# JuanTarrio/rebvo

Measured on AMD Instinct MI355X. Metric: frames/sec (DoG+extract+track+depth) 752x480 EuRoC, higher is better.
Workload: dtype f32 scale-space / f64 tracker+EKF

## Files before the change

### rebvo_amd/csrc/api.hip

```cpp

#include <math.h>
#include <stdio.h>
#include <stdlib.h>
#include <string.h>

#include <algorithm>
#include <mutex>

#include "ctx.h"
#include "stage_a_dev.h"

namespace edgehip {

static thread_local std::string g_err;

int wait_pinned_ring(edgehip_ctx *c) {
    const int r = c->frames_seen % 8;
    if (c->ring_valid[r]) EH_CHECK(hipEventSynchronize(c->ev_ring[r]));
    return 0;
}

static int wait_idx_row(edgehip_ctx *c, int slot, const int32_t *pi) {
    if (c->slot_src[slot].idx_row != pi) return 0;
    if (c->a_api_valid[slot]) EH_CHECK(hipEventSynchronize(c->ev_a[slot]));
// ... 379 lines not shown
        c->use_valid[i] = false;
    }
    EH_CHECK(hipEventCreateWithFlags(&c->ev_tmp, hipEventDisableTiming));
    EH_CHECK(hipEventCreateWithFlags(&c->ev_stage, hipEventDisableTiming));
    EH_CHECK(hipEventCreateWithFlags(&c->ev_stage8, hipEventDisableTiming));
    for (int i = 0; i < 8; i++) { EH_CHECK(hipEventCreateWithFlags(&c->ev_ring[i], hipEventDisableTiming)); c->ring_valid[i] = false; }
    if (nslots > 4) { set_error("edgehip_create: at most 4 frame slots"); return EDGEHIP_ERR_ARG; }

    DevicePlan &pl = c->plan;
    pl.w = p.w; pl.h = p.h; pl.n = p.w * p.h; pl.nseq = nseq; pl.nslots = nslots;
    pl.ftx = (p.w + 3) / 4;
    pl.fstride = (size_t)pl.ftx * (size_t)((p.h + 3) / 4) * 16;
    pl.f16tx = (p.w + 7) / 8;
    pl.f16stride = (size_t)pl.f16tx * (size_t)((p.h + 3) / 4) * 32;
    pl.cap = std::min(p.max_points, EDGEHIP_KEYLINE_MAX);
    const double sr0 = kovesi_boxes(p.sigma0, kMaxBoxes, pl.box[0]);
    kovesi_boxes(sr0 * p.ksigma, kMaxBoxes, pl.box[1]);
    for (int f = 0; f < 2; f++)
        for (int i = 0; i < kMaxBoxes; i++) {
            if (pl.box[f][i] < 1 || pl.box[f][i] * pl.box[f][i] >= kDivLutMax) {
                set_error("edgehip_create: box width out of range for these sigmas");
                return EDGEHIP_ERR_ARG;
            }
            pl.box_a[f][i] = (float)(1.0 / (pl.box[f][i] * pl.box[f][i]));
        }
    pl.ppx = (float)p.ppx; pl.ppy = (float)p.ppy; pl.zfx = (float)p.zfx; pl.zfy = (float)p.zfy;
    pl.zfm = (double)((pl.zfx + pl.zfy) / 2);

    const size_t B = nseq, S = nslots, N = pl.n, CAP = pl.cap;
    int e;
#define EH_TRY(x) if ((e = (x)) != 0) return e
    EH_TRY(dmalloc(c, &c->rgb, S * B * N * 3 + 16, al->dev, 0));
    EH_TRY(dmalloc(c, &c->ii, 4 * B * N, al->dev, 0));
    c->planes = nullptr;
    if (p.debug_planes) EH_TRY(dmalloc(c, &c->planes, 5 * B * N, al->dev, 0));
    EH_TRY(dmalloc(c, &c->mask, S * B * N, al->dev, 0xFF));
    EH_TRY(dmalloc(c, &c->field, B * pl.fstride, al->dev, 0xFF));
    EH_TRY(dmalloc(c, &c->field16, B * pl.f16stride, al->dev, 0));
    c->field32_valid = false;
    c->und_base = nullptr;
    c->und_iw = nullptr;
    if (p.use_undistort) {
        EH_TRY(dmalloc(c, &c->und_base, N, al->dev));
        EH_TRY(dmalloc(c, &c->und_iw, N, al->dev));
        std::vector<int32_t> base;
        std::vector<uint32_t> iw;
        build_undistort_map(p, base, iw, nullptr, nullptr);
        EH_CHECK(hipMemcpy(c->und_base, base.data(), sizeof(int32_t) * N, hipMemcpyHostToDevice));
        EH_CHECK(hipMemcpy(c->und_iw, iw.data(), sizeof(uint32_t) * 4 * N, hipMemcpyHostToDevice));
    }
    EH_TRY(dmalloc(c, &c->div_lut, kDivLutMax, al->dev));
    EH_TRY(dmalloc(c, &c->pinv, 3 * 49, al->dev, 0));
    EH_TRY(dmalloc(c, &c->seq, B, al->dev, 0));
    EH_TRY(dmalloc(c, &c->seqa, B, al->dev, 0));
    EH_TRY(dmalloc(c, &c->tresh_slot, S * B, al->dev, 0));
    c->fc_rows = std::max<int>(nslots, kRefRing);
    c->fc_index = 0;
    EH_TRY(dmalloc(c, &c->framecount, (size_t)c->fc_rows * B, al->dev, 0));
    EH_TRY(dmalloc(c, &c->kn_slot, S * B, al->dev, 0));
    EH_TRY(dmalloc(c, &c->retuned_slot, S * B, al->dev, 0));
    c->band_rows = detect_band_rows(p.w, p.plane_fit_size);
    c->nbands = (p.h - 2 * p.plane_fit_size + c->band_rows - 1) / c->band_rows;
    {
        const int npx = c->band_rows * p.w, nchunk = (npx + 63) / 64, cpw = (nchunk + kDetWaves - 1) / kDetWaves;
        c->band_cap = cpw * 64;
    }
    const size_t nstrips = (size_t)c->nbands * kDetWaves;
    EH_TRY(dmalloc(c, &c->band_cnt, B * nstrips, al->dev, 0));
    EH_TRY(dmalloc(c, &c->band_off, B * (nstrips + 1), al->dev, 0));
    {
        char *bs;
        EH_TRY(dmalloc(c, &bs, B * nstrips * c->band_cap * 20, al->dev));
        c->band_stage = bs;
    }
    EH_TRY(dmalloc(c, &c->histo, B * 256, al->dev, 0));
    c->nblk_tvr = (int)((CAP + kTvrBlock - 1) / kTvrBlock);
    EH_TRY(dmalloc(c, &c->P0, B * 3 * CAP, al->dev, 0));
    EH_TRY(dmalloc(c, &c->resid, (size_t)kResidBufs * B * CAP, al->dev, 0));
    EH_TRY(dmalloc(c, &c->resid_carry, (size_t)kResidBufs * B * c->nblk_tvr, al->dev, 0));
    EH_TRY(dmalloc(c, &c->partials, 2 * B * c->nblk_tvr * kNumSums, al->dev, 0));
    EH_TRY(dmalloc(c, &c->block_last, 2 * B * c->nblk_tvr, al->dev, 0));
    EH_TRY(dmalloc(c, &c->bin_cnt, B * 256, al->dev, 0));
    {
        const size_t ntiles = (size_t)((p.w + 63) / 64) * ((p.h + 63) / 64);
        EH_TRY(dmalloc(c, &c->bins, B * ntiles * CAP, al->dev));
    }
    c->field_radius = p.search_range;
    c->field_mode = EH_EXP_ENV("EDGEHIP_FIELD_MODE", 0);
    c->no_grec = getenv("EDGEHIP_NO_GREC") && atoi(getenv("EDGEHIP_NO_GREC")) != 0;
    c->level_mode = getenv("EDGEHIP_LEVEL_MODE") ? atoi(getenv("EDGEHIP_LEVEL_MODE")) : 0;
    c->fwd_mode = EH_EXP_ENV("EDGEHIP_FWD_MODE", 0);
    c->fused_min_batch = fused_min_env;
    c->fused_undist = EH_EXP_ENV("EDGEHIP_FUSED_UNDIST", 0) != 0;
    c->tvr_rw2 = EH_EXP_ENV("EDGEHIP_TVR_RW2", 0);
    c->dual_init = getenv("EDGEHIP_DUAL_INIT") ? atoi(getenv("EDGEHIP_DUAL_INIT")) : 1;
    c->persist_lm_max = EH_EXP_ENV("EDGEHIP_PERSIST_LM", 0);
    EH_TRY(dmalloc(c, &c->sync_cnt, B, al->dev, 0));
    EH_TRY(dmalloc(c, &c->fwd_key, B * CAP, al->dev, 0));
    EH_TRY(dmalloc(c, &c->fwd_win, B * CAP, al->dev, 0xFF));
    EH_TRY(dmalloc(c, &c->rs_tmp, B * 2 * CAP, al->dev, 0));
    c->fuse_match = !(getenv("EDGEHIP_FUSE_MATCH") && atoi(getenv("EDGEHIP_FUSE_MATCH")) == 0);
    if (c->fuse_match) {
        EH_TRY(dmalloc(c, &c->rot_pm, S * B * CAP, al->dev, 0)); EH_TRY(dmalloc(c, &c->rot_mm, S * B * CAP, al->dev, 0));
        EH_TRY(dmalloc(c, &c->rot_rho, S * B * CAP, al->dev, 0)); EH_TRY(dmalloc(c, &c->rot_srho, S * B * CAP, al->dev, 0));
    }
    EH_TRY(dmalloc(c, &c->rot_buf, B * 9, al->dev, 0));
    EH_TRY(dmalloc(c, &c->nav_dev, B, al->dev, 0));
    EH_TRY(dmalloc(c, &c->idx_dev, B, al->dev, 0));
    c->slot_src.assign(S, edgehip_ctx::SlotSrc());
    c->stereo_cnt = nullptr;
    if (p.stereo_available) EH_TRY(dmalloc(c, &c->stereo_cnt, B, al->dev, 0));
    c->nav_log = nullptr;
    c->nav_log_len = 0;

    {
        const size_t al256 = 256;
        auto up = [&](size_t x) { return (x + al256 - 1) / al256 * al256; };
        const bool stereo = p.stereo_available != 0;
        const size_t per = up(CAP * 4) * 8  +
                           up(CAP * 8) * 6  + up(CAP * 8) * 7  + up(CAP * 32) + up(CAP * 16)  +
                           (stereo ? up(CAP * 4) + 2 * up(CAP * 8) : 0);
        char *arena;
        EH_TRY(dmalloc(c, &arena, per * S * B, al->dev, 0));
        c->kl_arena = arena;
        c->kl.resize(S * B);
        for (size_t sb = 0; sb < S * B; sb++) {
            char *q = arena + sb * per;
            KlSoA &k = c->kl[sb];
            auto take = [&](size_t bytes) { char *r = q; q += up(bytes); return r; };
            k.p_inx = (int32_t *)take(CAP * 4);
            k.m_m = (float2 *)take(CAP * 8); k.u_m = (float2 *)take(CAP * 8); k.c_p = (float2 *)take(CAP * 8);
            k.p_m = (float2 *)take(CAP * 8); k.p_m_0 = (float2 *)take(CAP * 8); k.m_m0 = (float2 *)take(CAP * 8);
            k.n_m = (float *)take(CAP * 4);
            k.rho = (double *)take(CAP * 8); k.s_rho = (double *)take(CAP * 8); k.rho_nr = (double *)take(CAP * 8);
            k.s_rho_nr = (double *)take(CAP * 8); k.rho0 = (double *)take(CAP * 8); k.s_rho0 = (double *)take(CAP * 8);
            k.n_m0 = (double *)take(CAP * 8);
            k.m_id = (int32_t *)take(CAP * 4); k.m_id_f = (int32_t *)take(CAP * 4); k.m_id_kf = (int32_t *)take(CAP * 4);
            k.m_num = (int32_t *)take(CAP * 4); k.p_id = (int32_t *)take(CAP * 4); k.n_id = (int32_t *)take(CAP * 4);
            k.rec = (MatchRec *)take(CAP * 32);
            k.grec = (float4 *)take(CAP * 16);
            k.stereo_m_id = nullptr; k.stereo_rho = nullptr; k.stereo_s_rho = nullptr;
            if (stereo) {
                k.stereo_m_id = (int32_t *)take(CAP * 4);
                k.stereo_rho = (double *)take(CAP * 8); k.stereo_s_rho = (double *)take(CAP * 8);
            }
        }
        c->slot_cam.assign(S, edgehip_ctx::SlotCam{pl.ppx, pl.ppy, pl.zfm});
        EH_TRY(dmalloc(c, &c->kl_dev, S * B, al->dev));
        EH_CHECK(hipMemcpyAsync(c->kl_dev, c->kl.data(), sizeof(KlSoA) * S * B, hipMemcpyHostToDevice, c->stream));
    }
    {
        std::vector<float> lut(kDivLutMax, 0.f);
        for (int k = 1; k < kDivLutMax; k++) lut[k] = (float)(1.0 / (double)(float)k);
        EH_CHECK(hipMemcpyAsync(c->div_lut, lut.data(), sizeof(float) * kDivLutMax, hipMemcpyHostToDevice, c->stream));
        double pinv[3 * 49] = {0};
        plane_fit_pinv(p.plane_fit_size, pinv);
        if (p.plane_fit_size == 2)
            for (int i = 0; i < 5; i++)
                for (int j = 0; j < 5; j++) {
                    const int k = i * 5 + j;
                    if (!(pinv[k] == pinv[j] && pinv[25 + k] == pinv[25 + 5 * i] && pinv[50 + k] == pinv[50])) {
                        set_error("edgehip_create: plane-fit pseudo inverse lost its separable structure");
                        return EDGEHIP_ERR_STATE;
                    }
                }
        memcpy(c->pinv_host, pinv, sizeof c->pinv_host);
        EH_CHECK(hipMemcpyAsync(c->pinv, pinv, sizeof pinv, hipMemcpyHostToDevice, c->stream));
// ... 979 lines not shown
```

### rebvo_amd/csrc/ctx.h

```cpp
#pragma once
#include <hip/hip_runtime.h>
#include <stdint.h>
#include <string.h>
#include <string>
#include <map>
#include <vector>
#include <mutex>
#include <atomic>

#include "edgehip.h"
#include "export_ring.h"

namespace edgehip {

constexpr int kMaxBoxes = 3;
constexpr int kBandRows = 12;
constexpr int kDetWaves = 16;
constexpr int kDivLutMax = 256;
constexpr int kTvrThreads = 256;
constexpr int kTvrBlock = kTvrThreads;
constexpr int kNumSums = 28;
constexpr int kRefRing = 8;
constexpr int kResidBufs = 3;

__host__ __device__ inline uint64_t resid_carry_bits() { return 0x7FF8C0DEC0DEC0DEull; }

struct __attribute__((aligned(16))) MatchRec {
    float c_px, c_py, u_mx, u_my, m_mx, m_my, n_m, pad;
};

struct KlSoA {
    int32_t *p_inx;
    float2 *m_m, *u_m, *c_p, *p_m, *p_m_0, *m_m0;
    float *n_m;
    double *rho, *s_rho, *rho_nr, *s_rho_nr, *rho0, *s_rho0, *n_m0;
    int32_t *m_id, *m_id_f, *m_id_kf, *m_num, *p_id, *n_id;
    MatchRec *rec;
    float4 *grec;
    int32_t *stereo_m_id;
    double *stereo_rho, *stereo_s_rho;
};

struct SeqDev {
    edgehip_seq_state pub;
    int32_t kn_new;
    int32_t band_trunc;
    float nm_max, nm_min;
    double tresh_used;
    double X[6], Xnew[6], Xt[6], h[6];
    double JtJ[36], JtF[6], JtJnew[36], JtFnew[6];
    double F, Fnew, F0, Ft, F0t, u, v, ut, vt, gain;
    int32_t eff_steps, eff_steps_t, res_cur, res_new, res_t, lm_phase;
    int32_t kn_old, pad1;
    double s_rho_min_eval;
    double Rt[9], Vt[3], RM[4];
    int32_t nmatch_tmp, kf_tmp;
    double zX[6], zXnew[6], zh[6];
    double zJtJ[36], zJtF[6], zJtJnew[36], zJtFnew[6];
    double zF, zFnew, zF0, zu, zv, zgain;
    double zRt[9], zVt[3], zRM[4];
    int32_t z_eff_steps, z_pad;
    double mv_V[3], mv_Vnew[3], mv_h[3], mv_JtJ[9], mv_JtF[3], mv_JtJnew[9], mv_JtFnew[3], mv_RVel[9];
    double mv_F, mv_Fnew, mv_u, mv_v, mv_s_rho_min;
    float mv_min_mod; int32_t mv_pad;
    int32_t skip_match, skip_map;
    double t_cur;
    double V_track[3], W_track[3], PV_track[9], PW_track[9];
};

struct SeqA {
    double tresh;
    double tresh_used;
    int32_t l_kl_num;
    int32_t kn_new;
    int32_t band_trunc, pad0;
    float nm_max, nm_min;
    float retuned, pad1;
};

struct DevicePlan {
    int w, h, n, cap, nseq, nslots;
    int ftx;
    size_t fstride;
    int f16tx;
    size_t f16stride;
    int box[2][kMaxBoxes];
    float box_a[2][kMaxBoxes];
    float ppx, ppy, zfx, zfy;
    double zfm;
};

__device__ __forceinline__ int x86_cvttsd2si(double f) {
    if (!(f > -2147483649.0 && f < 2147483648.0)) return (int)0x80000000;
    return (int)f;
}

__device__ __forceinline__ int cvt_trunc_sat_i32(double f) {
    int r;
    asm("v_cvt_i32_f64 %0, %1" : "=v"(r) : "v"(f));
    return r;
}

#ifndef EDGEHIP_FASTDIV
#define EDGEHIP_FASTDIV 1
#endif
__device__ __forceinline__ double rcp_nr(const double b) {
// ... 528 lines not shown
```

### rebvo_amd/csrc/stage_b.hip

```cpp

#include <math.h>
#include <string.h>

#include <vector>

#include <type_traits>

#include "ctx.h"
#include "resid_carry.h"
#include "wave_reduce.h"

namespace edgehip {

struct RetuneArgs {
    SeqA *seqa;
    const int32_t *histo;
    float *retuned_out;
    int knum, nbins;
};
template <int NT>
__global__ __launch_bounds__(NT) void k_quantile(const KlSoA *kls, const int32_t *__restrict__ kns, SeqDev *seqs,
                                                 double smin, double smax, double pct, int nbins, const double *__restrict__ t_in, double fps,
                                                 RetuneArgs rt) {
    __shared__ int s_h[256];
// ... 99 lines not shown
constexpr int FT = 64;
constexpr int FG = 12;

__global__ __launch_bounds__(256) void k_field_tiles(const KlSoA *kls, const int32_t *__restrict__ masks,
                                                     const float *__restrict__ retuned, uint32_t *__restrict__ field,
                                                     int w, int h, size_t fstride, int ftx, int radius, float min_mod_arg) {
    __shared__ uint32_t s_tile[FT * FT];
    __shared__ int s_list[4096];
    __shared__ int s_cnt;
    const int seq = blockIdx.z, tid = threadIdx.x, lane = tid & 63;
    const int tx0 = blockIdx.x * FT, ty0 = blockIdx.y * FT;
    const KlSoA &k = kls[seq];
    const int32_t *mask = masks + (size_t)seq * ((size_t)w * h);
    const float min_mod = min_mod_arg < 0.f ? retuned[seq] : min_mod_arg;
    for (int i = tid; i < FT * FT; i += 256) s_tile[i] = 0xFFFFFFFFu;
    if (tid == 0) s_cnt = 0;
    const int rx0 = max(tx0 - radius - 1, 0), rx1 = min(tx0 + FT + radius + 1, w);
    const int ry0 = max(ty0 - radius - 1, 0), ry1 = min(ty0 + FT + radius + 1, h);
    const int rw = rx1 - rx0;
    const int rows_per_fill = max(1, min(FG, 4096 / rw));
    __syncthreads();
    for (int yg = ry0; yg < ry1; yg += rows_per_fill) {
        const int ye = min(yg + rows_per_fill, ry1);
        const int npx = (ye - yg) * rw;
        for (int base = 0; base < npx; base += 256) {
            const int idx = base + tid;
            int id = -1;
            if (idx < npx) {
                const int yy = yg + idx / rw, xx = rx0 + idx % rw;
                id = mask[(size_t)yy * w + xx];
            }
            const unsigned long long bal = __ballot(id >= 0);
            int wbase = 0;
            if (lane == 0 && bal) wbase = atomicAdd(&s_cnt, __popcll(bal));
            wbase = __shfl(wbase, 0, 64);
            if (id >= 0) s_list[wbase + __popcll(bal & ((1ull << lane) - 1ull))] = id;
        }
        __syncthreads();
        const int cnt = s_cnt;
        for (int li = tid; li < cnt; li += 256) {
            const int ikl = s_list[li];
            const MatchRec r = k.rec[ikl];
            if (min_mod > 0 && r.n_m < min_mod) continue;
            float tlo = (float)(-radius), thi = (float)(radius - 1);
            const float bx0 = (float)tx0 - 1.f - r.c_px, bx1 = (float)(tx0 + FT) - r.c_px;
            const float by0 = (float)ty0 - 1.f - r.c_py, by1 = (float)(ty0 + FT) - r.c_py;
            if (fabsf(r.u_mx) > 1e-6f) {
                const float a = bx0 / r.u_mx, b = bx1 / r.u_mx;
                tlo = fmaxf(tlo, fminf(a, b) - 1.f);
                thi = fminf(thi, fmaxf(a, b) + 1.f);
            } else if (bx0 > 0.f || bx1 < 0.f) continue;
            if (fabsf(r.u_my) > 1e-6f) {
                const float a = by0 / r.u_my, b = by1 / r.u_my;
                tlo = fmaxf(tlo, fminf(a, b) - 1.f);
                thi = fminf(thi, fmaxf(a, b) + 1.f);
            } else if (by0 > 0.f || by1 < 0.f) continue;
            const int t0 = (int)floorf(tlo), t1 = (int)ceilf(thi);
            const uint32_t idk = (uint32_t)(0xFFFF - ikl);
            for (int t = max(t0, -radius); t <= min(t1, radius - 1); t++) {
                const float fx = r.u_mx * (float)t + r.c_px;
                const float fy = r.u_my * (float)t + r.c_py;
                const int xi = round_half_away_i(fx), yi = round_half_away_i(fy);
                if (xi >= w || yi >= h || xi < 0 || yi < 0) continue;
                const int lx = xi - tx0, ly = yi - ty0;
                if ((unsigned)lx >= (unsigned)FT || (unsigned)ly >= (unsigned)FT) continue;
                const uint32_t at = (uint32_t)(t < 0 ? -t : t);
                atomicMin(&s_tile[ly * FT + lx], (at << 16) | idk);
            }
        }
        __syncthreads();
        if (tid == 0) s_cnt = 0;
        __syncthreads();
    }
    uint32_t *out = field + (size_t)seq * fstride;
    for (int i = tid; i < FT * FT; i += 256) {
        const int st = i >> 4, in = i & 15;
        const int lx = ((st % (FT / 4)) << 2) | (in & 3), ly = ((st / (FT / 4)) << 2) | (in >> 2);
        const int x = tx0 + lx, y = ty0 + ly;
        if (x < w && y < h) out[field_index(x, y, ftx)] = s_tile[ly * FT + lx];
    }
}

constexpr int kMaxTiles = 256;

__device__ __forceinline__ bool tile_trange(const MatchRec &r, int tx0, int ty0, int radius, int &t0, int &t1) {
    float tlo = (float)(-radius), thi = (float)(radius - 1);
    const float bx0 = (float)tx0 - 0.51f - r.c_px, bx1 = (float)(tx0 + FT) - 0.49f - r.c_px;
    const float by0 = (float)ty0 - 0.51f - r.c_py, by1 = (float)(ty0 + FT) - 0.49f - r.c_py;
    if (fabsf(r.u_mx) > 1e-6f) {
        const float iu = __builtin_amdgcn_rcpf(r.u_mx);
        const float a = bx0 * iu, b = bx1 * iu, sl = 0.25f + 1e-4f * fabsf(iu);
        tlo = fmaxf(tlo, fminf(a, b) - sl);
        thi = fminf(thi, fmaxf(a, b) + sl);
    } else if (bx0 > 0.f || bx1 < 0.f) return false;
    if (fabsf(r.u_my) > 1e-6f) {
        const float iu = __builtin_amdgcn_rcpf(r.u_my);
        const float a = by0 * iu, b = by1 * iu, sl = 0.25f + 1e-4f * fabsf(iu);
        tlo = fmaxf(tlo, fminf(a, b) - sl);
        thi = fminf(thi, fmaxf(a, b) + sl);
    } else if (by0 > 0.f || by1 < 0.f) return false;
    t0 = max((int)ceilf(tlo), -radius);
    t1 = min((int)floorf(thi), radius - 1);
    return t0 <= t1;
}

constexpr int kPackedRadiusMax = 127;
constexpr int kRngSlots = 9;

__device__ __forceinline__ uint32_t pack_trange(int t0, int t1, int radius) {
    return (uint32_t)(t0 + radius) | ((uint32_t)(t1 + radius) << 8);
}

template <bool PACKED>
__global__ __launch_bounds__(256) void k_field_bin(const KlSoA *kls, const int32_t *__restrict__ kns,
                                                   const float *__restrict__ retuned, int32_t *__restrict__ bin_cnt,
                                                   int32_t *__restrict__ bins, int w, int h, int radius, float min_mod_arg,
                                                   int ntx, int nty, int bin_cap, unsigned long long *__restrict__ fwd_key,
                                                   int32_t *__restrict__ fwd_win) {
    __shared__ int s_cnt[kMaxTiles], s_base[kMaxTiles];
    __shared__ uint16_t s_rng[PACKED ? kRngSlots * 256 : 1];
    const int seq = blockIdx.z, tid = threadIdx.x;
    const int i = blockIdx.x * 256 + tid;
    const int kn = kns[seq];
    if (blockIdx.x * 256 >= kn) return;

    const int ntiles = ntx * nty;
    for (int t = tid; t < ntiles; t += 256) s_cnt[t] = 0;
    __syncthreads();
    bool active = i < kn;
    MatchRec r;
    int txa = 0, txb = -1, tya = 0, tyb = -1;
    if (active) {
        r = kls[seq].rec[i];
        const float min_mod = min_mod_arg < 0.f ? retuned[seq] : min_mod_arg;
        if (min_mod > 0 && r.n_m < min_mod) active = false;
    }
    if (active) {
        const float rr = (float)radius + 1.5f;
        const float xa = r.c_px - fabsf(r.u_mx) * rr - 1.f, xb = r.c_px + fabsf(r.u_mx) * rr + 1.f;
        const float ya = r.c_py - fabsf(r.u_my) * rr - 1.f, yb = r.c_py + fabsf(r.u_my) * rr + 1.f;
        txa = max((int)floorf(xa) / FT, 0); txb = min((int)floorf(xb) / FT, ntx - 1);
        tya = max((int)floorf(ya) / FT, 0); tyb = min((int)floorf(yb) / FT, nty - 1);
        if (xb < 0.f || yb < 0.f) txb = -1;
    }
    const int bw = txb - txa + 1;
    const bool cached = bw > 0 && (tyb - tya + 1) * bw <= (PACKED ? kRngSlots : 32);
    uint32_t hitmask = 0;
    for (int ty = tya; ty <= tyb; ty++)
        for (int tx = txa; tx <= txb; tx++) {
            int t0, t1;
            const bool hit = tile_trange(r, tx * FT, ty * FT, radius, t0, t1);
            if (hit) atomicAdd(&s_cnt[ty * ntx + tx], 1);
            if constexpr (PACKED) {
                if (cached) s_rng[((ty - tya) * bw + (tx - txa)) * 256 + tid] = hit ? (uint16_t)pack_trange(t0, t1, radius) : (uint16_t)0xFFFFu;
            } else {
                if (hit && cached) hitmask |= 1u << ((ty - tya) * bw + (tx - txa));
            }
        }
    __syncthreads();
    for (int t = tid; t < ntiles; t += 256) {
        const int c = s_cnt[t];
        s_base[t] = c ? atomicAdd(&bin_cnt[(size_t)seq * kMaxTiles + t], c) : 0;
        s_cnt[t] = 0;
    }
    __syncthreads();
    for (int ty = tya; ty <= tyb; ty++)
        for (int tx = txa; tx <= txb; tx++) {
            int t0, t1;
            bool hit;
            uint32_t entry = (uint32_t)i;
            if constexpr (PACKED) {
                uint32_t rng;
                if (cached) { rng = s_rng[((ty - tya) * bw + (tx - txa)) * 256 + tid]; hit = rng != 0xFFFFu; }
                else { hit = tile_trange(r, tx * FT, ty * FT, radius, t0, t1); rng = hit ? pack_trange(t0, t1, radius) : 0u; }
                entry |= rng << 16;
            } else {
                hit = cached ? ((hitmask >> ((ty - tya) * bw + (tx - txa))) & 1u) != 0u : tile_trange(r, tx * FT, ty * FT, radius, t0, t1);
            }
            if (hit) {
                const int t = ty * ntx + tx;
                const int pos = s_base[t] + atomicAdd(&s_cnt[t], 1);
                if (pos < bin_cap) bins[((size_t)seq * ntiles + t) * bin_cap + pos] = (int32_t)entry;
            }
        }
    if (fwd_key && i < kn) { fwd_key[(size_t)seq * bin_cap + i] = 0ull; fwd_win[(size_t)seq * bin_cap + i] = -1; }
}

#ifndef EDGEHIP_NT_RASTER
#define EDGEHIP_NT_RASTER 1
#endif
template <bool PACKED>
__global__ __launch_bounds__(256) void k_field_raster(const KlSoA *kls, int32_t *__restrict__ bin_cnt,
                                                      const int32_t *__restrict__ bins, uint32_t *__restrict__ field,
                                                      uint16_t *__restrict__ field16, size_t f16stride, int f16tx, int keep32,
                                                      int w, int h, size_t fstride, int ftx, int radius, int ntx, int bin_cap) {
#ifndef EDGEHIP_RASTER_PAD
#define EDGEHIP_RASTER_PAD 2
#endif
    constexpr int TS = FT + EDGEHIP_RASTER_PAD;
    __shared__ uint32_t s_tile[FT * TS];
    const int ntiles = ntx * gridDim.y;
    const int seq = blockIdx.z, tid = threadIdx.x;
    const int tx0 = blockIdx.x * FT, ty0 = blockIdx.y * FT;
    const int tile = blockIdx.y * ntx + blockIdx.x;
    for (int i = tid; i < FT * TS; i += 256) s_tile[i] = 0xFFFFFFFFu;
    __syncthreads();
    const int cnt = min(bin_cnt[(size_t)seq * kMaxTiles + tile], bin_cap);
    const int32_t *list = bins + ((size_t)seq * ntiles + tile) * bin_cap;
    const KlSoA &k = kls[seq];
    const unsigned ex = (unsigned)min(FT, w - tx0), ey = (unsigned)min(FT, h - ty0);
#ifndef EDGEHIP_FSPLIT
#define EDGEHIP_FSPLIT 2
#endif
#ifndef EDGEHIP_RASTER_ABL
#define EDGEHIP_RASTER_ABL 0
#endif
#ifndef EDGEHIP_RASTER_UNROLL
#define EDGEHIP_RASTER_UNROLL 2
#endif
    constexpr int FSPLIT = EDGEHIP_FSPLIT;
    const unsigned ex4 = ex << 2;
    const int neg4tx0 = -4 * tx0;
    const unsigned org = (unsigned)(neg4tx0 - ty0 * (TS * 4));
    const float radius_f = (float)radius;
    auto raster = [&](auto fix_x, auto fix_y) {
        for (int wi = tid; wi < cnt * FSPLIT; wi += 256) {
            const int li = wi / FSPLIT, part = wi - li * FSPLIT;
            const uint32_t entry = (uint32_t)list[li];
            const int ikl = PACKED ? (int)(entry & 0xFFFFu) : (int)entry;
#if EDGEHIP_RASTER_ABL >= 5
            MatchRec r;
            r.c_px = (float)(tx0 + (ikl & 63)); r.c_py = (float)(ty0 + ((ikl >> 6) & 63)); r.u_mx = 0.6f; r.u_my = 0.8f;
#else
            MatchRec r;
            { const float4 q = ldg(reinterpret_cast<const float4 *>(k.rec), 2 * (size_t)ikl); r.c_px = q.x; r.c_py = q.y; r.u_mx = q.z; r.u_my = q.w; }
#endif
            float lo, hi;
            if constexpr (PACKED) {
                lo = (float)((entry >> 16) & 0xFFu) - radius_f;
                hi = (float)(entry >> 24) - radius_f;
            } else {
                int t0, t1;
                if (!tile_trange(r, tx0, ty0, radius, t0, t1)) continue;
                lo = (float)t0; hi = (float)t1;
            }
#ifndef EDGEHIP_RASTER_PK
#define EDGEHIP_RASTER_PK 0
#endif
#if EDGEHIP_RASTER_PK
            typedef float v2f __attribute__((ext_vector_type(2)));
            const v2f u2 = {r.u_mx, r.u_my}, c2 = {r.c_px, r.c_py};
#endif
            auto at = [&](const float tf, float &fx, float &fy) __attribute__((always_inline)) {
#if EDGEHIP_RASTER_PK
                const v2f t2 = {tf, tf};
                const v2f f2 = u2 * t2 + c2;
                fx = f2.x; fy = f2.y;
#else
                fx = r.u_mx * tf + r.c_px;
                fy = r.u_my * tf + r.c_py;
#endif
            };
            auto inside = [&](const float tf) __attribute__((always_inline)) -> bool {
                float fx, fy;
                at(tf, fx, fy);
                const int rx = decltype(fix_x)::value ? round_half_away_i(fx) : round_ties_up_i(fx);
                const int ry = decltype(fix_y)::value ? round_half_away_i(fy) : round_ties_up_i(fy);
                return (unsigned)((rx << 2) + neg4tx0) < ex4 && (unsigned)(ry - ty0) < ey;
            };
            if constexpr (FSPLIT == 2) {
                const float step = part ? -1.f : 1.f;
                float tf = part ? hi : lo;
                for (float n = hi - lo; n >= 0.f && !inside(tf); n -= 1.f) tf += step;
                const float other = __int_as_float(__builtin_amdgcn_update_dpp(0, __float_as_int(tf), 0xB1, 0xf, 0xf, true));
                lo = part ? other : tf;
                hi = part ? tf : other;
            } else {
                while (lo <= hi && !inside(lo)) lo += 1.f;
                while (hi > lo && !inside(hi)) hi -= 1.f;
            }
            if (lo > hi) continue;
            int t0 = (int)lo, t1 = (int)hi;
            {
                const int chunk = (t1 - t0 + FSPLIT) / FSPLIT;
                t0 += part * chunk;
                t1 = min(t1, t0 + chunk - 1);
            }
            const uint32_t idk = (uint32_t)(0xFFFF - ikl);
#if EDGEHIP_RASTER_ABL == 2
            uint32_t acc_abl = 0;
#endif
#if EDGEHIP_RASTER_ABL >= 3
            if (t0 == 12345) s_tile[0] = idk;
            continue;
#endif
            auto sample = [&](const float tf) __attribute__((always_inline)) {
                float fx, fy;
                at(tf, fx, fy);
                const unsigned off = ((unsigned)round_ties_up_i(fx) << 2) + (__umul24((unsigned)round_ties_up_i(fy), (unsigned)(TS * 4)) + org);
                const uint32_t val = __builtin_amdgcn_cvt_pk_u8_f32(fabsf(tf), 2u, idk);
                uint32_t *const px = reinterpret_cast<uint32_t *>(reinterpret_cast<char *>(s_tile) + off);
#if EDGEHIP_RASTER_ABL == 1
                *px = val;
#elif EDGEHIP_RASTER_ABL == 2
                acc_abl += val | off;
#else
                atomicMin(px, val);
#endif
            };
            constexpr int UNROLL = EDGEHIP_RASTER_UNROLL;
            const float t1f = (float)t1;
            float tf = (float)t0;
            if constexpr (UNROLL > 1) {
                for (; tf + (float)(UNROLL - 1) <= t1f; tf += (float)UNROLL) {
#pragma unroll
                    for (int j = 0; j < UNROLL; j++) sample(tf + (float)j);
                }
            }
            for (; tf <= t1f; tf += 1.f) sample(tf);
#if EDGEHIP_RASTER_ABL == 2
            if (acc_abl == 0x12345u) s_tile[1] = acc_abl;
#endif
        }
    };
    using T = std::true_type;
    using F = std::false_type;
    if (tx0 == 0) { if (ty0 == 0) raster(T{}, T{}); else raster(T{}, F{}); }
    else { if (ty0 == 0) raster(F{}, T{}); else raster(F{}, F{}); }
    __syncthreads();
    if (tid == 0) bin_cnt[(size_t)seq * kMaxTiles + tile] = 0;
#if EDGEHIP_RASTER_ABL == 4
    if (s_tile[tid] != 0x12345u) return;
#endif
    if (keep32) {
        uint32_t *out = field + (size_t)seq * fstride;
        for (int i = tid; i < FT * FT; i += 256) {
            const int st = i >> 4, in = i & 15;
            const int lx = ((st % (FT / 4)) << 2) | (in & 3), ly = ((st / (FT / 4)) << 2) | (in >> 2);
            const int x = tx0 + lx, y = ty0 + ly;
            if (x < w && y < h) out[field_index(x, y, ftx)] = s_tile[ly * TS + lx];
        }
    }
    uint16_t *o16 = field16 + (size_t)seq * f16stride;
    for (int i = tid; i < FT * FT / 2; i += 256) {
        const int st = i >> 4, in = i & 15;
        const int lx = ((st % (FT / 8)) << 3) | ((in & 3) << 1), ly = ((st / (FT / 8)) << 2) | (in >> 2);
        const int x = tx0 + lx, y = ty0 + ly;
        if (x < w && y < h) {
            const uint32_t v0 = s_tile[ly * TS + lx], v1 = s_tile[ly * TS + lx + 1];
            const uint32_t a0 = v0 == 0xFFFFFFFFu ? 0u : ((0x10000u - (v0 & 0xFFFFu)) & 0xFFFFu);
            const uint32_t a1 = v1 == 0xFFFFFFFFu ? 0u : ((0x10000u - (v1 & 0xFFFFu)) & 0xFFFFu);
#if EDGEHIP_NT_RASTER
            st_stream(reinterpret_cast<uint32_t *>(o16 + field16_index(x, y, f16tx)), a0 | (a1 << 16));
#else
            *reinterpret_cast<uint32_t *>(o16 + field16_index(x, y, f16tx)) = a0 | (a1 << 16);
#endif
        }
    }
}

__global__ __launch_bounds__(256) void k_field_to16(const uint32_t *__restrict__ field, uint16_t *__restrict__ f16, int w, int h,
                                                    size_t fstride, int ftx, size_t f16stride, int f16tx) {
    const int seq = blockIdx.z;
    const size_t e = (size_t)blockIdx.x * 256 + threadIdx.x;
    if (e >= f16stride) return;
    const size_t tile = e >> 5; const int in = (int)(e & 31);
    const int x = (int)(tile % (size_t)f16tx) * 8 + (in & 7), y = (int)(tile / (size_t)f16tx) * 4 + (in >> 3);
    uint16_t v = 0;
    if (x < w && y < h) {
        const uint32_t f = field[(size_t)seq * fstride + field_index(x, y, ftx)];
        if (f != 0xFFFFFFFFu) v = (uint16_t)(0xFFFF - (int)(f & 0xFFFFu) + 1);
    }
    f16[(size_t)seq * f16stride + e] = v;
}

__global__ __launch_bounds__(256) void k_tvr_prepare(const KlSoA *kls, const int32_t *__restrict__ kns, double *__restrict__ P0,
                                                     double *__restrict__ resid0, double *__restrict__ carry0, SeqDev *seqs,
                                                     int cap, int nblk, double zfm) {
    const int seq = blockIdx.z;
    const int i = blockIdx.x * 256 + threadIdx.x;
    const int kn = kns[seq];
    if (i == 0) seqs[seq].kn_old = kn;
    if ((i % kTvrBlock) == 0 && i / kTvrBlock < nblk) carry0[(size_t)seq * nblk + i / kTvrBlock] = 0.0;
    if (i >= kn) return;
    resid0[(size_t)seq * cap + i] = 0.0;
}

__device__ __forceinline__ void so3_exp_inl(const double (&w)[3], double (&R)[9]) {
    const double one_6th = 1.0 / 6.0, one_20th = 1.0 / 20.0;
    const double theta_sq = w[0] * w[0] + w[1] * w[1] + w[2] * w[2];
    const double theta = sqrt(theta_sq);
    double A, B;
    if (theta_sq < 1e-8) {
        A = 1.0 - one_6th * theta_sq;
        B = 0.5;
    } else if (theta_sq < 1e-6) {
        B = 0.5 - 0.25 * one_6th * theta_sq;
        A = 1.0 - theta_sq * one_6th * (1.0 - one_20th * theta_sq);
    } else {
        const double inv_theta = 1.0 / theta;
        A = sin(theta) * inv_theta;
        B = (1 - cos(theta)) * (inv_theta * inv_theta);
    }
    const double wx2 = w[0] * w[0], wy2 = w[1] * w[1], wz2 = w[2] * w[2];
    R[0] = 1.0 - B * (wy2 + wz2);
    R[4] = 1.0 - B * (wx2 + wz2);
    R[8] = 1.0 - B * (wx2 + wy2);
    double a = A * w[2], b = B * (w[0] * w[1]);
    R[1] = b - a; R[3] = b + a;
    a = A * w[1]; b = B * (w[0] * w[2]);
    R[2] = b + a; R[6] = b - a;
    a = A * w[0]; b = B * (w[1] * w[2]);
    R[5] = b - a; R[7] = b + a;
}
__device__ __noinline__ void so3_exp(const double w[3], double R[9]) {
    const double wv[3] = {w[0], w[1], w[2]};
    double Rr[9];
    so3_exp_inl(wv, Rr);
    for (int i = 0; i < 9; i++) R[i] = Rr[i];
}

__device__ __noinline__ void tvr_setup(SeqDev *sq, const double *X) {
    double R0[9], Rz[9];
    so3_exp(X + 3, R0);
    const double wz[3] = {0.0, 0.0, X[5]};
    so3_exp(wz, Rz);
    for (int i = 0; i < 9; i++) sq->Rt[i] = R0[i];
    sq->RM[0] = Rz[0]; sq->RM[1] = Rz[1]; sq->RM[2] = Rz[3]; sq->RM[3] = Rz[4];
    for (int i = 0; i < 3; i++) sq->Vt[i] = X[i];
// ... 1921 lines not shown
#pragma unroll
        for (int i = 0; i < 3; i++) den += (0.5 * h[i]) * (u * h[i] - JtF[i]);
        const double gain = (F - Fnew) / den;
        if (gain > 0) {
            F = Fnew;
#pragma unroll
            for (int i = 0; i < 3; i++) { V[i] = Vn[i]; JtF[i] = JtFn[i]; }
#pragma unroll
            for (int i = 0; i < 9; i++) JtJ[i] = JtJn[i];
            const double g = 2 * gain - 1;
            const double m = 1 - (g * g * g);
            u *= (0.33 > m ? 0.33 : m);
            v = 2;
        } else {
            u *= v;
            v *= 2;
        }
    }
    if (ops & LMV_SOLVE) {
        double ApI[9], Inv[9];
#pragma unroll
        for (int i = 0; i < 9; i++) ApI[i] = JtJ[i] + ((i % 4 == 0) ? 1.0 * u : 0.0);
        mat3_inv(ApI, Inv);
#pragma unroll
        for (int i = 0; i < 3; i++) {
            double d = 0;
#pragma unroll
            for (int k = 0; k < 3; k++) d += Inv[i * 3 + k] * (-JtF[k]);
            h[i] = d;
            Vn[i] = V[i] + d;
        }
    }
    double RVel[9];
    if (ops & LMV_FINISH) mat3_inv(JtJ, RVel);
#pragma unroll
    for (int i = 0; i < 3; i++) { sq->mv_V[i] = V[i]; sq->mv_Vnew[i] = Vn[i]; sq->mv_h[i] = h[i]; sq->mv_JtF[i] = JtF[i]; sq->mv_JtFnew[i] = JtFn[i]; }
#pragma unroll
    for (int i = 0; i < 9; i++) { sq->mv_JtJ[i] = JtJ[i]; sq->mv_JtJnew[i] = JtJn[i]; }
    sq->mv_F = F; sq->mv_Fnew = Fnew; sq->mv_u = u; sq->mv_v = v;
    if (ops & LMV_FINISH) {
#pragma unroll
        for (int i = 0; i < 9; i++) sq->mv_RVel[i] = RVel[i];
    }
}

__global__ void k_tvr_setup_from_host(SeqDev *seqs, const double *__restrict__ X, const double *__restrict__ smin, int nseq,
                                      int res_in, int res_out) {
    const int seq = blockIdx.x * blockDim.x + threadIdx.x;
    if (seq >= nseq) return;
    SeqDev *sq = seqs + seq;
    double x[6];
    for (int i = 0; i < 6; i++) x[i] = X[seq * 6 + i];
    tvr_setup(sq, x);
    sq->s_rho_min_eval = smin[seq];
    sq->res_cur = res_in < 0 ? 0 : res_in;
    sq->res_new = res_out;
    sq->lm_phase = 1;
}

int quantile_enqueue(edgehip_ctx *c, int slot, double smin, double smax, double pct, int nbins, bool frame_begins, int retune_slot) {
    RetuneArgs rt = {};
    if (retune_slot >= 0) {
        rt.seqa = c->seqa; rt.histo = c->histo; rt.retuned_out = c->retuned_slot + (size_t)retune_slot * c->plan.nseq;
        rt.knum = c->p.track_points; rt.nbins = c->p.qcut_nbins;
    }
    ProfScope ps(c, PROF_B_QUANTILE);
    if (nbins < 1 || nbins > 256) { set_error("quantile: 1 <= nbins <= 256"); return EDGEHIP_ERR_ARG; }
    if (c->plan.nseq <= 64)
        hipLaunchKernelGGL(k_quantile<1024>, dim3(c->plan.nseq), dim3(1024), 0, c->stream, kldev(c, slot),
                           c->kn_slot + (size_t)slot * c->plan.nseq, c->seq, smin, smax, pct, nbins, frame_begins ? c->t_src : (const double *)nullptr, c->p.config_fps, rt);
    else
        hipLaunchKernelGGL(k_quantile<256>, dim3(c->plan.nseq), dim3(256), 0, c->stream, kldev(c, slot),
                           c->kn_slot + (size_t)slot * c->plan.nseq, c->seq, smin, smax, pct, nbins, frame_begins ? c->t_src : (const double *)nullptr, c->p.config_fps, rt);
    EH_LAUNCH_CHECK();
    return 0;
}

int build_field_enqueue(edgehip_ctx *c, int slot, int radius, float min_mod, bool clear_fwd) {
    c->fwd_cleared = false;
    ProfScope ps(c, PROF_B_FIELD);
    const DevicePlan &pl = c->plan;
    if (radius < 1 || radius > 255) { set_error("build_field: 1 <= radius <= 255"); return EDGEHIP_ERR_ARG; }
    c->field_radius = radius;
    const int ntx = (pl.w + FT - 1) / FT, nty = (pl.h + FT - 1) / FT;
    if (c->field_mode == 0 && ntx * nty <= kMaxTiles) {
#ifndef EDGEHIP_FIELD_PACKED_RANGE
#define EDGEHIP_FIELD_PACKED_RANGE 1
#endif
        const bool packed = EDGEHIP_FIELD_PACKED_RANGE && radius <= kPackedRadiusMax && pl.cap <= 65536;
        auto bin = packed ? k_field_bin<true> : k_field_bin<false>;
        auto raster = packed ? k_field_raster<true> : k_field_raster<false>;
        hipLaunchKernelGGL(bin, dim3((pl.cap + 255) / 256, 1, pl.nseq), dim3(256), 0, c->stream, kldev(c, slot),
                           c->kn_slot + (size_t)slot * pl.nseq, c->retuned_slot + (size_t)slot * pl.nseq, c->bin_cnt, c->bins,
                           pl.w, pl.h, radius, min_mod, ntx, nty, pl.cap, clear_fwd ? c->fwd_key : nullptr, clear_fwd ? c->fwd_win : nullptr);
        c->fwd_cleared = clear_fwd;
        hipLaunchKernelGGL(raster, dim3(ntx, nty, pl.nseq), dim3(256), 0, c->stream, kldev(c, slot), c->bin_cnt,
                           c->bins, c->field, c->field16, pl.f16stride, pl.f16tx, c->p.debug_planes ? 1 : 0, pl.w, pl.h,
                           pl.fstride, pl.ftx, radius, ntx, pl.cap);
        c->field32_valid = c->p.debug_planes != 0;
        EH_LAUNCH_CHECK();
        return 0;
    } else if (c->field_mode == 2 || c->field_mode == 0) {
        hipLaunchKernelGGL(k_field_tiles, dim3((pl.w + FT - 1) / FT, (pl.h + FT - 1) / FT, pl.nseq), dim3(256), 0, c->stream,
                           kldev(c, slot), maskof(c, slot), c->retuned_slot + (size_t)slot * pl.nseq, c->field, pl.w, pl.h,
                           pl.fstride, pl.ftx, radius, min_mod);
    } else {
#ifdef EDGEHIP_EXPERIMENTS
        EH_CHECK(hipMemsetAsync(c->field, 0xFF, sizeof(uint32_t) * pl.nseq * pl.fstride, c->stream));
        const long long threads = (long long)pl.cap * 2 * radius;
        hipLaunchKernelGGL(k_field_scatter, dim3((unsigned)((threads + 255) / 256), 1, pl.nseq), dim3(256), 0, c->stream,
                           kldev(c, slot), c->kn_slot + (size_t)slot * pl.nseq, c->retuned_slot + (size_t)slot * pl.nseq,
                           c->field, pl.w, pl.h, pl.fstride, pl.ftx, radius, min_mod);
#else
        set_error("build_field: unknown field mode");
        return EDGEHIP_ERR_STATE;
#endif
    }
    EH_LAUNCH_CHECK();
    hipLaunchKernelGGL(k_field_to16, dim3((unsigned)((pl.f16stride + 255) / 256), 1, pl.nseq), dim3(256), 0, c->stream, c->field,
                       c->field16, pl.w, pl.h, pl.fstride, pl.ftx, pl.f16stride, pl.f16tx);
    c->field32_valid = true;
    EH_LAUNCH_CHECK();
    return 0;
}

int tvr_prepare_enqueue(edgehip_ctx *c, int slot_old, unsigned begin_ops) {
    ProfScope ps(c, PROF_B_PREP);
    const DevicePlan &pl = c->plan;
    if (begin_ops) {
        LmArgs l;
        l.seq = c->seq; l.partials = c->partials; l.block_last = c->block_last; l.resid_carry = c->resid_carry;
        l.framecount = c->framecount + (size_t)c->fc_index * pl.nseq;
        l.nblk = c->nblk_tvr; l.nseq = pl.nseq; l.ops = begin_ops; l.init_type = c->p.tracker_init_type;
        l.kf_in = c->kf_req_dev; l.kf_out = c->kf_res_dev;
        l.kn_src = c->kn_slot + (size_t)slot_old * pl.nseq;
        l.f32 = c->tracker_f32 ? 1 : 0;
        hipLaunchKernelGGL(k_tvr_prepare_begin, dim3((pl.cap + 255) / 256, 1, pl.nseq), dim3(256), 0, c->stream, l.kn_src, c->resid,
                           c->resid_carry, pl.cap, c->nblk_tvr, l);
        EH_LAUNCH_CHECK();
        return 0;
    }
    hipLaunchKernelGGL(k_tvr_prepare, dim3((pl.cap + 255) / 256, 1, pl.nseq), dim3(256), 0, c->stream, kldev(c, slot_old),
                       c->kn_slot + (size_t)slot_old * pl.nseq, c->P0, c->resid, c->resid_carry, c->seq, pl.cap,
                       c->nblk_tvr, pl.zfm);
    EH_LAUNCH_CHECK();
    return 0;
}

static TvrArgs make_tvr_args(edgehip_ctx *c, int slot_new, int slot_old, double match_thresh, double k_huber,
                             uint32_t match_num_thresh, int write_mid) {
    const DevicePlan &pl = c->plan;
    TvrArgs a;
    a.kl_old = kldev(c, slot_old); a.kl_new = kldev(c, slot_new);
    a.kn_old = c->kn_slot + (size_t)slot_old * pl.nseq;
    a.field16 = c->field16; a.f16stride = pl.f16stride; a.f16tx = pl.f16tx; a.P0 = c->P0; a.resid = c->resid; a.resid_carry = c->resid_carry;
    a.block_last = c->block_last; a.partials = c->partials; a.seq = c->seq;
    a.block_last_z = c->block_last + (size_t)pl.nseq * c->nblk_tvr;
    a.partials_z = c->partials + (size_t)pl.nseq * c->nblk_tvr * kNumSums;
    a.framecount = c->framecount + (size_t)c->fc_index * pl.nseq;
    a.w = pl.w; a.h = pl.h; a.cap = pl.cap; a.nblk = c->nblk_tvr; a.nseq = pl.nseq;
    a.zfm = pl.zfm; a.inv_zfm = 1.0 / pl.zfm; a.max_r = (double)c->field_radius; a.match_thresh = match_thresh; a.k_huber = k_huber; a.inv_k_huber = 1.0 / k_huber;
    a.ppx = pl.ppx; a.ppy = pl.ppy; a.match_num_thresh = match_num_thresh; a.write_mid = write_mid;
    a.use_grec = c->grec_ok[slot_new] && !c->no_grec;
    a.kf = nullptr; a.kf_match_mod = a.kf_match_cang = a.kf_rho_tol = 0;
    a.fwd_key = (write_mid && c->fwd_key_in_tvr) ? c->fwd_key : nullptr;
    return a;
}

static int launch_tvr(edgehip_ctx *c, const TvrArgs &a, bool reweight, bool procjf) {
    ProfScope ps(c, PROF_B_TRYVELROT);
    dim3 g(c->nblk_tvr, 1, c->plan.nseq), b(kTvrThreads);
#ifdef EDGEHIP_EXPERIMENTS
    if (reweight && procjf && c->tvr_rw2 && (size_t)c->nblk_tvr * c->plan.nseq >= (size_t)c->tvr_rw2) {
        dim3 g2((c->nblk_tvr + 1) / 2, 1, c->plan.nseq);
        if (a.use_grec) hipLaunchKernelGGL((k_try_velrot_rw2<true>), g2, b, 0, c->stream, a);
        else hipLaunchKernelGGL((k_try_velrot_rw2<false>), g2, b, 0, c->stream, a);
        EH_LAUNCH_CHECK();
        return 0;
    }
// ... 450 lines not shown
```

Measured before the change: 134,200.

## Enlarge field rasterization tiles to 128x128 and hoist per-match reciprocals

Decouples the field binning and raster tile size from the 64-px FT constant and raises it to 128x128, with 1024 threads per raster block. Larger tiles mean each match segment lands in fewer bins, which cuts binning atomics and duplicated per-tile raster work. The reciprocals of the match direction are now computed once per match instead of on every tile-range test. In exchange, the grid has far fewer blocks (6x4 per sequence at 752x480), which may underfill the GPU at small batch sizes, and the shared tile grows to about 66KB.

After: 134,800, median of 3. About the same (+0.5%).

```diff
diff --git a/rebvo_amd/csrc/api.hip b/rebvo_amd/csrc/api.hip
--- a/rebvo_amd/csrc/api.hip
+++ b/rebvo_amd/csrc/api.hip
@@ -485,7 +485,7 @@
     EH_TRY(dmalloc(c, &c->block_last, 2 * B * c->nblk_tvr, al->dev, 0));
     EH_TRY(dmalloc(c, &c->bin_cnt, B * 256, al->dev, 0));
     {
-        const size_t ntiles = (size_t)((p.w + 63) / 64) * ((p.h + 63) / 64);
+        const size_t ntiles = (size_t)((p.w + kFieldTW - 1) / kFieldTW) * ((p.h + kFieldTH - 1) / kFieldTH);
         EH_TRY(dmalloc(c, &c->bins, B * ntiles * CAP, al->dev));
     }
     c->field_radius = p.search_range;
diff --git a/rebvo_amd/csrc/ctx.h b/rebvo_amd/csrc/ctx.h
--- a/rebvo_amd/csrc/ctx.h
+++ b/rebvo_amd/csrc/ctx.h
@@ -22,6 +22,18 @@
 constexpr int kNumSums = 28;
 constexpr int kRefRing = 8;
 constexpr int kResidBufs = 3;
+
+#ifndef EDGEHIP_FIELD_TW
+#define EDGEHIP_FIELD_TW 128
+#endif
+#ifndef EDGEHIP_FIELD_TH
+#define EDGEHIP_FIELD_TH 128
+#endif
+constexpr int kFieldTW = EDGEHIP_FIELD_TW, kFieldTH = EDGEHIP_FIELD_TH;
+constexpr int kFieldRasterThreads = kFieldTW * kFieldTH / 16;
+static_assert(kFieldTW % 8 == 0 && kFieldTH % 4 == 0, "the rasteriser stores whole 4x4 and 8x4 output tiles");
+static_assert(kFieldTW >= 64 && kFieldTH >= 64 && kFieldTW <= 128 && kFieldTH <= 128, "a +-127 segment spans at most 3 x 3 tiles; one block per tile");
+static_assert(kFieldRasterThreads % 64 == 0 && kFieldRasterThreads <= 1024, "whole waves, one block");
 
 __host__ __device__ inline uint64_t resid_carry_bits() { return 0x7FF8C0DEC0DEC0DEull; }
 
diff --git a/rebvo_amd/csrc/stage_b.hip b/rebvo_amd/csrc/stage_b.hip
--- a/rebvo_amd/csrc/stage_b.hip
+++ b/rebvo_amd/csrc/stage_b.hip
@@ -205,20 +205,28 @@
 }
 
 constexpr int kMaxTiles = 256;
-
-__device__ __forceinline__ bool tile_trange(const MatchRec &r, int tx0, int ty0, int radius, int &t0, int &t1) {
+constexpr int TW = kFieldTW, TH = kFieldTH;
+constexpr int kRasterThreads = kFieldRasterThreads;
+
+struct TrangeInv { float iux, iuy, slx, sly; };
+__device__ __forceinline__ TrangeInv trange_inv(const MatchRec &r) {
+    TrangeInv v;
+    v.iux = __builtin_amdgcn_rcpf(r.u_mx); v.slx = 0.25f + 1e-4f * fabsf(v.iux);
+    v.iuy = __builtin_amdgcn_rcpf(r.u_my); v.sly = 0.25f + 1e-4f * fabsf(v.iuy);
+    return v;
+}
+
+__device__ __forceinline__ bool tile_trange(const MatchRec &r, const TrangeInv &v, int tx0, int ty0, int radius, int &t0, int &t1) {
     float tlo = (float)(-radius), thi = (float)(radius - 1);
-    const float bx0 = (float)tx0 - 0.51f - r.c_px, bx1 = (float)(tx0 + FT) - 0.49f - r.c_px;
-    const float by0 = (float)ty0 - 0.51f - r.c_py, by1 = (float)(ty0 + FT) - 0.49f - r.c_py;
+    const float bx0 = (float)tx0 - 0.51f - r.c_px, bx1 = (float)(tx0 + TW) - 0.49f - r.c_px;
+    const float by0 = (float)ty0 - 0.51f - r.c_py, by1 = (float)(ty0 + TH) - 0.49f - r.c_py;
     if (fabsf(r.u_mx) > 1e-6f) {
-        const float iu = __builtin_amdgcn_rcpf(r.u_mx);
-        const float a = bx0 * iu, b = bx1 * iu, sl = 0.25f + 1e-4f * fabsf(iu);
+        const float a = bx0 * v.iux, b = bx1 * v.iux, sl = v.slx;
         tlo = fmaxf(tlo, fminf(a, b) - sl);
         thi = fminf(thi, fmaxf(a, b) + sl);
     } else if (bx0 > 0.f || bx1 < 0.f) return false;
     if (fabsf(r.u_my) > 1e-6f) {
-        const float iu = __builtin_amdgcn_rcpf(r.u_my);
-        const float a = by0 * iu, b = by1 * iu, sl = 0.25f + 1e-4f * fabsf(iu);
+        const float a = by0 * v.iuy, b = by1 * v.iuy, sl = v.sly;
         tlo = fmaxf(tlo, fminf(a, b) - sl);
         thi = fminf(thi, fmaxf(a, b) + sl);
     } else if (by0 > 0.f || by1 < 0.f) return false;
@@ -262,17 +270,18 @@
         const float rr = (float)radius + 1.5f;
         const float xa = r.c_px - fabsf(r.u_mx) * rr - 1.f, xb = r.c_px + fabsf(r.u_mx) * rr + 1.f;
         const float ya = r.c_py - fabsf(r.u_my) * rr - 1.f, yb = r.c_py + fabsf(r.u_my) * rr + 1.f;
-        txa = max((int)floorf(xa) / FT, 0); txb = min((int)floorf(xb) / FT, ntx - 1);
-        tya = max((int)floorf(ya) / FT, 0); tyb = min((int)floorf(yb) / FT, nty - 1);
+        txa = max((int)floorf(xa) / TW, 0); txb = min((int)floorf(xb) / TW, ntx - 1);
+        tya = max((int)floorf(ya) / TH, 0); tyb = min((int)floorf(yb) / TH, nty - 1);
         if (xb < 0.f || yb < 0.f) txb = -1;
     }
+    const TrangeInv inv = trange_inv(r);
     const int bw = txb - txa + 1;
     const bool cached = bw > 0 && (tyb - tya + 1) * bw <= (PACKED ? kRngSlots : 32);
     uint32_t hitmask = 0;
     for (int ty = tya; ty <= tyb; ty++)
         for (int tx = txa; tx <= txb; tx++) {
             int t0, t1;
-            const bool hit = tile_trange(r, tx * FT, ty * FT, radius, t0, t1);
+            const bool hit = tile_trange(r, inv, tx * TW, ty * TH, radius, t0, t1);
             if (hit) atomicAdd(&s_cnt[ty * ntx + tx], 1);
             if constexpr (PACKED) {
                 if (cached) s_rng[((ty - tya) * bw + (tx - txa)) * 256 + tid] = hit ? (uint16_t)pack_trange(t0, t1, radius) : (uint16_t)0xFFFFu;
@@ -295,10 +304,10 @@
             if constexpr (PACKED) {
                 uint32_t rng;
                 if (cached) { rng = s_rng[((ty - tya) * bw + (tx - txa)) * 256 + tid]; hit = rng != 0xFFFFu; }
-                else { hit = tile_trange(r, tx * FT, ty * FT, radius, t0, t1); rng = hit ? pack_trange(t0, t1, radius) : 0u; }
+                else { hit = tile_trange(r, inv, tx * TW, ty * TH, radius, t0, t1); rng = hit ? pack_trange(t0, t1, radius) : 0u; }
                 entry |= rng << 16;
             } else {
-                hit = cached ? ((hitmask >> ((ty - tya) * bw + (tx - txa))) & 1u) != 0u : tile_trange(r, tx * FT, ty * FT, radius, t0, t1);
+                hit = cached ? ((hitmask >> ((ty - tya) * bw + (tx - txa))) & 1u) != 0u : tile_trange(r, inv, tx * TW, ty * TH, radius, t0, t1);
             }
             if (hit) {
                 const int t = ty * ntx + tx;
@@ -313,25 +322,25 @@
 #define EDGEHIP_NT_RASTER 1
 #endif
 template <bool PACKED>
-__global__ __launch_bounds__(256) void k_field_raster(const KlSoA *kls, int32_t *__restrict__ bin_cnt,
+__global__ __launch_bounds__(kRasterThreads) void k_field_raster(const KlSoA *kls, int32_t *__restrict__ bin_cnt,
                                                       const int32_t *__restrict__ bins, uint32_t *__restrict__ field,
                                                       uint16_t *__restrict__ field16, size_t f16stride, int f16tx, int keep32,
                                                       int w, int h, size_t fstride, int ftx, int radius, int ntx, int bin_cap) {
 #ifndef EDGEHIP_RASTER_PAD
 #define EDGEHIP_RASTER_PAD 2
 #endif
-    constexpr int TS = FT + EDGEHIP_RASTER_PAD;
-    __shared__ uint32_t s_tile[FT * TS];
+    constexpr int TS = TW + EDGEHIP_RASTER_PAD;
+    __shared__ uint32_t s_tile[TH * TS];
     const int ntiles = ntx * gridDim.y;
     const int seq = blockIdx.z, tid = threadIdx.x;
-    const int tx0 = blockIdx.x * FT, ty0 = blockIdx.y * FT;
+    const int tx0 = blockIdx.x * TW, ty0 = blockIdx.y * TH;
     const int tile = blockIdx.y * ntx + blockIdx.x;
-    for (int i = tid; i < FT * TS; i += 256) s_tile[i] = 0xFFFFFFFFu;
+    for (int i = tid; i < TH * TS; i += kRasterThreads) s_tile[i] = 0xFFFFFFFFu;
     __syncthreads();
     const int cnt = min(bin_cnt[(size_t)seq * kMaxTiles + tile], bin_cap);
     const int32_t *list = bins + ((size_t)seq * ntiles + tile) * bin_cap;
     const KlSoA &k = kls[seq];
-    const unsigned ex = (unsigned)min(FT, w - tx0), ey = (unsigned)min(FT, h - ty0);
+    const unsigned ex = (unsigned)min(TW, w - tx0), ey = (unsigned)min(TH, h - ty0);
 #ifndef EDGEHIP_FSPLIT
 #define EDGEHIP_FSPLIT 2
 #endif
@@ -347,7 +356,7 @@
     const unsigned org = (unsigned)(neg4tx0 - ty0 * (TS * 4));
     const float radius_f = (float)radius;
     auto raster = [&](auto fix_x, auto fix_y) {
-        for (int wi = tid; wi < cnt * FSPLIT; wi += 256) {
+        for (int wi = tid; wi < cnt * FSPLIT; wi += kRasterThreads) {
             const int li = wi / FSPLIT, part = wi - li * FSPLIT;
             const uint32_t entry = (uint32_t)list[li];
             const int ikl = PACKED ? (int)(entry & 0xFFFFu) : (int)entry;
@@ -364,7 +373,7 @@
                 hi = (float)(entry >> 24) - radius_f;
             } else {
                 int t0, t1;
-                if (!tile_trange(r, tx0, ty0, radius, t0, t1)) continue;
+                if (!tile_trange(r, trange_inv(r), tx0, ty0, radius, t0, t1)) continue;
                 lo = (float)t0; hi = (float)t1;
             }
 #ifndef EDGEHIP_RASTER_PK
@@ -457,17 +466,17 @@
 #endif
     if (keep32) {
         uint32_t *out = field + (size_t)seq * fstride;
-        for (int i = tid; i < FT * FT; i += 256) {
+        for (int i = tid; i < TW * TH; i += kRasterThreads) {
             const int st = i >> 4, in = i & 15;
-            const int lx = ((st % (FT / 4)) << 2) | (in & 3), ly = ((st / (FT / 4)) << 2) | (in >> 2);
+            const int lx = ((st % (TW / 4)) << 2) | (in & 3), ly = ((st / (TW / 4)) << 2) | (in >> 2);
             const int x = tx0 + lx, y = ty0 + ly;
             if (x < w && y < h) out[field_index(x, y, ftx)] = s_tile[ly * TS + lx];
         }
     }
     uint16_t *o16 = field16 + (size_t)seq * f16stride;
-    for (int i = tid; i < FT * FT / 2; i += 256) {
+    for (int i = tid; i < TW * TH / 2; i += kRasterThreads) {
         const int st = i >> 4, in = i & 15;
-        const int lx = ((st % (FT / 8)) << 3) | ((in & 3) << 1), ly = ((st / (FT / 8)) << 2) | (in >> 2);
+        const int lx = ((st % (TW / 8)) << 3) | ((in & 3) << 1), ly = ((st / (TW / 8)) << 2) | (in >> 2);
         const int x = tx0 + lx, y = ty0 + ly;
         if (x < w && y < h) {
             const uint32_t v0 = s_tile[ly * TS + lx], v1 = s_tile[ly * TS + lx + 1];
@@ -2555,8 +2564,9 @@
     const DevicePlan &pl = c->plan;
     if (radius < 1 || radius > 255) { set_error("build_field: 1 <= radius <= 255"); return EDGEHIP_ERR_ARG; }
     c->field_radius = radius;
-    const int ntx = (pl.w + FT - 1) / FT, nty = (pl.h + FT - 1) / FT;
-    if (c->field_mode == 0 && ntx * nty <= kMaxTiles) {
+    const int ntx = (pl.w + TW - 1) / TW, nty = (pl.h + TH - 1) / TH;
+    static_assert(TW >= FT && TH >= FT, "ntx * nty <= kMaxTiles follows from the 64-px count");
+    if (c->field_mode == 0 && ((pl.w + FT - 1) / FT) * ((pl.h + FT - 1) / FT) <= kMaxTiles) {
 #ifndef EDGEHIP_FIELD_PACKED_RANGE
 #define EDGEHIP_FIELD_PACKED_RANGE 1
 #endif
@@ -2567,7 +2577,7 @@
                            c->kn_slot + (size_t)slot * pl.nseq, c->retuned_slot + (size_t)slot * pl.nseq, c->bin_cnt, c->bins,
                            pl.w, pl.h, radius, min_mod, ntx, nty, pl.cap, clear_fwd ? c->fwd_key : nullptr, clear_fwd ? c->fwd_win : nullptr);
         c->fwd_cleared = clear_fwd;
-        hipLaunchKernelGGL(raster, dim3(ntx, nty, pl.nseq), dim3(256), 0, c->stream, kldev(c, slot), c->bin_cnt,
+        hipLaunchKernelGGL(raster, dim3(ntx, nty, pl.nseq), dim3(kRasterThreads), 0, c->stream, kldev(c, slot), c->bin_cnt,
                            c->bins, c->field, c->field16, pl.f16stride, pl.f16tx, c->p.debug_planes ? 1 : 0, pl.w, pl.h,
                            pl.fstride, pl.ftx, radius, ntx, pl.cap);
         c->field32_valid = c->p.debug_planes != 0;
```
